# pytorch/ELF

Hardware: AMD Instinct MI355X
Metric: mcts_rollouts_per_sec (self-play, 19x19 Go, 8192 rollouts/move, bs 16) (higher is better)
Workload: dtype f32; 1 GPU; BASELINE configs[2]: MCTS self-play bs=16, 8192 rollouts/move, 20x256 fp16 net on PyTorch-ROCm, 2048 games/GPU in 1 group(s), window crosses a move boundary; games_per_gpu=2048, groups=1, board_size=19, mcts_threads=1, net_dtype=fp16, moves_in_window=2048, nodes_per_game=12288, node_bytes=6626, live_nodes=6241478, largest_tree=8184

## Files before the change

elf_amd/csrc/net_conv3x3.hip:

```cpp
#include <hip/hip_runtime.h>
#include <stdint.h>

#include "../../include/elf_amd.h"


namespace {

typedef _Float16 half8 __attribute__((ext_vector_type(8)));
typedef _Float16 half4 __attribute__((ext_vector_type(4)));
typedef float floatx16 __attribute__((ext_vector_type(16)));

constexpr int kTileM = 256;
constexpr int kTileN = 256;
constexpr int kThreads = 512;
constexpr int kOperandBytes = 256 * 128;
constexpr int kBufBytes = 2 * kOperandBytes;
constexpr int kLdsBytes = 2 * kBufBytes;

__device__ __attribute__((aligned(128))) unsigned char g_zero_line[128] = {0};

typedef const __attribute__((address_space(1))) void* gptr_t;
typedef __attribute__((address_space(3))) void* lptr_t;

__device__ __forceinline__ void stage16(const char* src, char* lds_base) {
  __builtin_amdgcn_global_load_lds((gptr_t)src, (lptr_t)lds_base, 16, 0, 0);
}

template <bool kHasRes>
__global__ __launch_bounds__(kThreads, 2) void k_conv3x3_f16(const char* __restrict__ x, const char* __restrict__ w,
                                                             const _Float16* __restrict__ bias, const _Float16* __restrict__ res,
                                                             _Float16* __restrict__ y, int M, int H, int W, int Cin, int K, int relu) {
  __shared__ __attribute__((aligned(128))) char lds[kLdsBytes];
  const int tid = threadIdx.x, lane = tid & 63, wv = tid >> 6;
  const int tile = blockIdx.x, kbase = blockIdx.y * kTileN;

  uint32_t xoff[4], woff[4], xmask[4];
  const unsigned char* zsrc = g_zero_line + (lane & 7) * 16;
#pragma unroll
  for (int i = 0; i < 4; ++i) {
    const int r = (i * 8 + wv) * 8 + (lane >> 3);
    const int chunk = (lane & 7) ^ ((r >> 1) & 7);
    const int p = tile * kTileM + r;
    uint32_t m = 0;
    if (p < M) {
      const int rem = p % (H * W), hh = rem / W, ww = rem - hh * W;
#pragma unroll
      for (int tap = 0; tap < 9; ++tap) {
        const int dy = tap / 3 - 1, dx = tap % 3 - 1;
        if ((unsigned)(hh + dy) < (unsigned)H && (unsigned)(ww + dx) < (unsigned)W) m |= 1u << tap;
      }
    }
    xmask[i] = m;
    xoff[i] = (uint32_t)p * (uint32_t)(Cin * 2) + chunk * 16;
    woff[i] = (uint32_t)(kbase + r) * (uint32_t)(9 * Cin * 2) + chunk * 16;
  }
  auto piece = [&](int j, int tap, int kc, int buf) {
    char* dst = lds + buf * kBufBytes + wv * 1024;
    if (j < 4) {
      const int dy = tap / 3 - 1, dx = tap - (tap / 3) * 3 - 1;
      const uint32_t d = (uint32_t)((dy * W + dx) * Cin * 2 + kc * 128);
      stage16(((xmask[j] >> tap) & 1) ? x + (uint32_t)(xoff[j] + d) : (const char*)zsrc, dst + j * 8192);
    } else {
      stage16(w + (uint32_t)(woff[j - 4] + (uint32_t)(tap * Cin * 2 + kc * 128)), dst + kOperandBytes + (j - 4) * 8192);
    }
  };

  const int wm = wv >> 2, wn = wv & 3;
  const int fr = lane & 31, fh = lane >> 5;
  const int sw = (fr >> 1) & 7;
  const int xrow = (wm * 128 + fr) * 128;
  const int wrow = kOperandBytes + (wn * 64 + fr) * 128;
  int cs[4];
#pragma unroll
  for (int kk = 0; kk < 4; ++kk) cs[kk] = (((kk >> 1) * 4 + fh * 2 + (kk & 1)) ^ sw) << 4;

  floatx16 acc[4][2];
#pragma unroll
  for (int mt = 0; mt < 4; ++mt)
#pragma unroll
    for (int nt = 0; nt < 2; ++nt)
#pragma unroll
      for (int e = 0; e < 16; ++e) acc[mt][nt][e] = 0.0f;

  const int kchunks = Cin >> 6, ktiles = 9 * kchunks;
#pragma unroll
  for (int j = 0; j < 8; ++j) piece(j, 0, 0, 0);
  int tap = 0, kc = 0;
  for (int t = 0; t < ktiles; ++t) {
    asm volatile("s_waitcnt vmcnt(0)" ::: "memory");
    __syncthreads();
    int ntap = tap, nkc = kc + 1;
    if (nkc == kchunks) { nkc = 0; ++ntap; }
    const bool more = t + 1 < ktiles;
    const int nbuf = (t + 1) & 1;
    tap = ntap; kc = nkc;
    const char* b = lds + (t & 1) * kBufBytes;
    half8 xf[2][4], wf[2][2];
#pragma unroll
    for (int nt = 0; nt < 2; ++nt) wf[0][nt] = *(const half8*)(b + wrow + nt * 4096 + cs[0]);
#pragma unroll
    for (int mt = 0; mt < 4; ++mt) xf[0][mt] = *(const half8*)(b + xrow + mt * 4096 + cs[0]);
#pragma unroll
    for (int kk = 0; kk < 4; ++kk) {
      const int cur = kk & 1, nxt = cur ^ 1;
      if (kk < 3) {
#pragma unroll
        for (int nt = 0; nt < 2; ++nt) wf[nxt][nt] = *(const half8*)(b + wrow + nt * 4096 + cs[kk + 1]);
#pragma unroll
        for (int mt = 0; mt < 4; ++mt) xf[nxt][mt] = *(const half8*)(b + xrow + mt * 4096 + cs[kk + 1]);
      }
      __builtin_amdgcn_sched_barrier(0);
#pragma unroll
      for (int mt = 0; mt < 2; ++mt)
#pragma unroll
        for (int nt = 0; nt < 2; ++nt)
          acc[mt][nt] = __builtin_amdgcn_mfma_f32_32x32x16_f16(wf[cur][nt], xf[cur][mt], acc[mt][nt], 0, 0, 0);
      __builtin_amdgcn_sched_barrier(0);
      if (more && kk < 2) { piece(4 * kk, ntap, nkc, nbuf); piece(4 * kk + 1, ntap, nkc, nbuf); }
      __builtin_amdgcn_sched_barrier(0);
#pragma unroll
      for (int mt = 2; mt < 4; ++mt)
#pragma unroll
        for (int nt = 0; nt < 2; ++nt)
          acc[mt][nt] = __builtin_amdgcn_mfma_f32_32x32x16_f16(wf[cur][nt], xf[cur][mt], acc[mt][nt], 0, 0, 0);
      __builtin_amdgcn_sched_barrier(0);
      if (more && kk < 2) { piece(4 * kk + 2, ntap, nkc, nbuf); piece(4 * kk + 3, ntap, nkc, nbuf); }
      __builtin_amdgcn_sched_barrier(0);
    }
  }

  __syncthreads();
#pragma unroll
  for (int mt = 0; mt < 4; ++mt)
#pragma unroll
    for (int nt = 0; nt < 2; ++nt) {
      const int pos = wm * 128 + mt * 32 + fr;
#pragma unroll
      for (int g = 0; g < 4; ++g) {
        const int ch = wn * 64 + nt * 32 + g * 8 + fh * 4;
        half4 hv;
#pragma unroll
        for (int e = 0; e < 4; ++e) hv[e] = (_Float16)acc[mt][nt][g * 4 + e];
        *(half4*)(lds + pos * 512 + (((ch >> 3) ^ (pos & 31)) << 4) + ((ch >> 2) & 1) * 8) = hv;
      }
    }
  const int q = tid & 31;
  const half8 bv = *(const half8*)(bias + kbase + q * 8);
  if constexpr (kHasRes) {
    half8 rv[16];
#pragma unroll
    for (int it = 0; it < 16; ++it) {
      const int p = tile * kTileM + it * 16 + (tid >> 5);
      rv[it] = *(const half8*)(res + (size_t)(p < M ? p : M - 1) * K + kbase + q * 8);
    }
    __syncthreads();
#pragma unroll
    for (int it = 0; it < 16; ++it) {
      const int pos = it * 16 + (tid >> 5);
      const int p = tile * kTileM + pos;
      const half8 cv = *(const half8*)(lds + pos * 512 + ((q ^ (pos & 31)) << 4));
      half8 ov;
#pragma unroll
      for (int e = 0; e < 8; ++e) {
        float v = (float)cv[e];
        v += (float)bv[e];
        v += (float)rv[it][e];
        if (relu) v = fmaxf(v, 0.0f);
        ov[e] = (_Float16)v;
      }
      if (p < M) *(half8*)(y + (size_t)p * K + kbase + q * 8) = ov;
    }
  } else {
    __syncthreads();
#pragma unroll 4
    for (int it = 0; it < 16; ++it) {
      const int pos = it * 16 + (tid >> 5);
      const int p = tile * kTileM + pos;
      if (p < M) {
        const half8 cv = *(const half8*)(lds + pos * 512 + ((q ^ (pos & 31)) << 4));
        half8 ov;
#pragma unroll
        for (int e = 0; e < 8; ++e) {
          float v = (float)cv[e];
          v += (float)bv[e];
          if (relu) v = fmaxf(v, 0.0f);
          ov[e] = (_Float16)v;
        }
        *(half8*)(y + (size_t)p * K + kbase + q * 8) = ov;
      }
    }
  }
}

}

extern "C" __attribute__((visibility("hidden"))) int elfnet_conv3x3_native_f16(const void* x, const void* w, const void* bias,
                                                                               const void* res, void* y, int64_t rows, int h, int wd,
                                                                               int c, int k, int relu, hipStream_t stream) {
  if ((c & 63) != 0 || (k & 255) != 0) return ELFGO_E_BADARG;
  const int64_t m = rows * h * wd;
  const dim3 grid((unsigned)((m + kTileM - 1) / kTileM), (unsigned)(k / kTileN));
  if (res)
    hipLaunchKernelGGL(k_conv3x3_f16<true>, grid, dim3(kThreads), 0, stream, (const char*)x, (const char*)w, (const _Float16*)bias,
                       (const _Float16*)res, (_Float16*)y, (int)m, h, wd, c, k, relu);
  else
    hipLaunchKernelGGL(k_conv3x3_f16<false>, grid, dim3(kThreads), 0, stream, (const char*)x, (const char*)w, (const _Float16*)bias,
                       (const _Float16*)nullptr, (_Float16*)y, (int)m, h, wd, c, k, relu);
  hipError_t e = hipGetLastError();
  return e == hipSuccess ? 0 : (int)e;
}
```

Measured before the change: 59540 rollouts/s.

## Restructure conv3x3 main loop into ping-pong staged pipeline with split wave groups

Rewrites the 3x3 conv GEMM main loop so that operand staging into LDS is split into half-tile pieces. The pieces are issued between two MFMA phases with partial vmcnt waits instead of a full drain each k-tile. The two wave halves are offset by one barrier, a ping-pong schedule in which one group computes while the other loads. MFMA sections run at raised priority, and the staging layout is remapped so each half of the tile arrives independently. This targets the load-wait stalls at every k-tile boundary, but the barrier and vmcnt logic is fragile and brings a risk of races or deadlock if the counts are wrong.

Result: faster. 61890 rollouts/s, median of 6 (+3.9%).

```diff
diff --git a/elf_amd/csrc/net_conv3x3.hip b/elf_amd/csrc/net_conv3x3.hip
--- a/elf_amd/csrc/net_conv3x3.hip
+++ b/elf_amd/csrc/net_conv3x3.hip
@@ -26,20 +26,33 @@
   __builtin_amdgcn_global_load_lds((gptr_t)src, (lptr_t)lds_base, 16, 0, 0);
 }
 
+template <int kN, bool kLgkm>
+__device__ __forceinline__ void wait_staged() {
+  if constexpr (kLgkm) asm volatile("s_waitcnt vmcnt(%0) lgkmcnt(0)" ::"n"(kN) : "memory");
+  else asm volatile("s_waitcnt vmcnt(%0)" ::"n"(kN) : "memory");
+}
+__device__ __forceinline__ void raw_barrier() {
+  __builtin_amdgcn_s_barrier();
+  asm volatile("" ::: "memory");
+  __builtin_amdgcn_sched_barrier(0);
+}
+template <int kV> struct Mode { static constexpr int v = kV; };
+
 template <bool kHasRes>
 __global__ __launch_bounds__(kThreads, 2) void k_conv3x3_f16(const char* __restrict__ x, const char* __restrict__ w,
                                                              const _Float16* __restrict__ bias, const _Float16* __restrict__ res,
                                                              _Float16* __restrict__ y, int M, int H, int W, int Cin, int K, int relu) {
   __shared__ __attribute__((aligned(128))) char lds[kLdsBytes];
-  const int tid = threadIdx.x, lane = tid & 63, wv = tid >> 6;
-  const int tile = blockIdx.x, kbase = blockIdx.y * kTileN;
+  const int tid = threadIdx.x, lane = tid & 63, wv = __builtin_amdgcn_readfirstlane(tid >> 6);
+  const int kbase = blockIdx.y * kTileN;
+  const int tile = blockIdx.x;
 
   uint32_t xoff[4], woff[4], xmask[4];
   const unsigned char* zsrc = g_zero_line + (lane & 7) * 16;
 #pragma unroll
-  for (int i = 0; i < 4; ++i) {
-    const int r = (i * 8 + wv) * 8 + (lane >> 3);
-    const int chunk = (lane & 7) ^ ((r >> 1) & 7);
+  for (int j = 0; j < 4; ++j) {
+    const int hf = j >> 1, i = j & 1;
+    const int r = i * 128 + hf * 64 + wv * 8 + (lane >> 3);
     const int p = tile * kTileM + r;
     uint32_t m = 0;
     if (p < M) {
@@ -50,19 +63,25 @@
         if ((unsigned)(hh + dy) < (unsigned)H && (unsigned)(ww + dx) < (unsigned)W) m |= 1u << tap;
       }
     }
-    xmask[i] = m;
-    xoff[i] = (uint32_t)p * (uint32_t)(Cin * 2) + chunk * 16;
-    woff[i] = (uint32_t)(kbase + r) * (uint32_t)(9 * Cin * 2) + chunk * 16;
+    xmask[j] = m;
+    xoff[j] = (uint32_t)p * (uint32_t)(Cin * 2) + (((lane & 7) ^ ((r >> 1) & 7)) << 4);
+    const int rw = (i * 2 + (wv >> 2)) * 64 + hf * 32 + (wv & 3) * 8 + (lane >> 3);
+    woff[j] = (uint32_t)(kbase + rw) * (uint32_t)(9 * Cin * 2) + (((lane & 7) ^ ((rw >> 1) & 7)) << 4);
   }
-  auto piece = [&](int j, int tap, int kc, int buf) {
-    char* dst = lds + buf * kBufBytes + wv * 1024;
-    if (j < 4) {
-      const int dy = tap / 3 - 1, dx = tap - (tap / 3) * 3 - 1;
-      const uint32_t d = (uint32_t)((dy * W + dx) * Cin * 2 + kc * 128);
-      stage16(((xmask[j] >> tap) & 1) ? x + (uint32_t)(xoff[j] + d) : (const char*)zsrc, dst + j * 8192);
-    } else {
-      stage16(w + (uint32_t)(woff[j - 4] + (uint32_t)(tap * Cin * 2 + kc * 128)), dst + kOperandBytes + (j - 4) * 8192);
-    }
+  auto stage_x = [&](int hf, int tap, int kc, int buf) {
+    const int dy = tap / 3 - 1, dx = tap - (tap / 3) * 3 - 1;
+    const uint32_t d = (uint32_t)((dy * W + dx) * Cin * 2 + kc * 128);
+#pragma unroll
+    for (int i = 0; i < 2; ++i)
+      stage16(((xmask[hf * 2 + i] >> tap) & 1) ? x + (uint32_t)(xoff[hf * 2 + i] + d) : (const char*)zsrc,
+              lds + buf * kBufBytes + (i * 128 + hf * 64 + wv * 8) * 128);
+  };
+  auto stage_w = [&](int hf, int tap, int kc, int buf) {
+    const uint32_t d = (uint32_t)(tap * Cin * 2 + kc * 128);
+#pragma unroll
+    for (int i = 0; i < 2; ++i)
+      stage16(w + (uint32_t)(woff[hf * 2 + i] + d),
+              lds + buf * kBufBytes + kOperandBytes + ((i * 2 + (wv >> 2)) * 64 + hf * 32 + (wv & 3) * 8) * 128);
   };
 
   const int wm = wv >> 2, wn = wv & 3;
@@ -73,6 +92,8 @@
   int cs[4];
 #pragma unroll
   for (int kk = 0; kk < 4; ++kk) cs[kk] = (((kk >> 1) * 4 + fh * 2 + (kk & 1)) ^ sw) << 4;
+  auto ldx = [&](const char* b, int mt, int kk) { return *(const half8*)(b + xrow + mt * 4096 + cs[kk]); };
+  auto ldw = [&](const char* b, int nt, int kk) { return *(const half8*)(b + wrow + nt * 4096 + cs[kk]); };
 
   floatx16 acc[4][2];
 #pragma unroll
@@ -83,51 +104,70 @@
       for (int e = 0; e < 16; ++e) acc[mt][nt][e] = 0.0f;
 
   const int kchunks = Cin >> 6, ktiles = 9 * kchunks;
-#pragma unroll
-  for (int j = 0; j < 8; ++j) piece(j, 0, 0, 0);
-  int tap = 0, kc = 0;
-  for (int t = 0; t < ktiles; ++t) {
-    asm volatile("s_waitcnt vmcnt(0)" ::: "memory");
-    __syncthreads();
-    int ntap = tap, nkc = kc + 1;
-    if (nkc == kchunks) { nkc = 0; ++ntap; }
-    const bool more = t + 1 < ktiles;
-    const int nbuf = (t + 1) & 1;
-    tap = ntap; kc = nkc;
-    const char* b = lds + (t & 1) * kBufBytes;
-    half8 xf[2][4], wf[2][2];
-#pragma unroll
-    for (int nt = 0; nt < 2; ++nt) wf[0][nt] = *(const half8*)(b + wrow + nt * 4096 + cs[0]);
-#pragma unroll
-    for (int mt = 0; mt < 4; ++mt) xf[0][mt] = *(const half8*)(b + xrow + mt * 4096 + cs[0]);
-#pragma unroll
-    for (int kk = 0; kk < 4; ++kk) {
-      const int cur = kk & 1, nxt = cur ^ 1;
-      if (kk < 3) {
-#pragma unroll
-        for (int nt = 0; nt < 2; ++nt) wf[nxt][nt] = *(const half8*)(b + wrow + nt * 4096 + cs[kk + 1]);
-#pragma unroll
-        for (int mt = 0; mt < 4; ++mt) xf[nxt][mt] = *(const half8*)(b + xrow + mt * 4096 + cs[kk + 1]);
-      }
-      __builtin_amdgcn_sched_barrier(0);
-#pragma unroll
-      for (int mt = 0; mt < 2; ++mt)
-#pragma unroll
-        for (int nt = 0; nt < 2; ++nt)
-          acc[mt][nt] = __builtin_amdgcn_mfma_f32_32x32x16_f16(wf[cur][nt], xf[cur][mt], acc[mt][nt], 0, 0, 0);
-      __builtin_amdgcn_sched_barrier(0);
-      if (more && kk < 2) { piece(4 * kk, ntap, nkc, nbuf); piece(4 * kk + 1, ntap, nkc, nbuf); }
-      __builtin_amdgcn_sched_barrier(0);
-#pragma unroll
-      for (int mt = 2; mt < 4; ++mt)
-#pragma unroll
-        for (int nt = 0; nt < 2; ++nt)
-          acc[mt][nt] = __builtin_amdgcn_mfma_f32_32x32x16_f16(wf[cur][nt], xf[cur][mt], acc[mt][nt], 0, 0, 0);
-      __builtin_amdgcn_sched_barrier(0);
-      if (more && kk < 2) { piece(4 * kk + 2, ntap, nkc, nbuf); piece(4 * kk + 3, ntap, nkc, nbuf); }
-      __builtin_amdgcn_sched_barrier(0);
-    }
+  half8 xf[2][4], wa[4], wb[4];
+  int tap1 = 0, kc1 = 1, tap2 = 0, kc2 = 2;
+  if (kchunks == 1) { tap1 = 1; kc1 = 0; tap2 = 2; kc2 = 0; }
+  else if (kchunks == 2) { tap2 = 1; kc2 = 0; }
+  stage_x(0, 0, 0, 0); stage_w(0, 0, 0, 0); stage_w(1, 0, 0, 0); stage_x(1, 0, 0, 0);
+  stage_x(0, tap1, kc1, 1); stage_w(0, tap1, kc1, 1); stage_w(1, tap1, kc1, 1);
+  wait_staged<8, false>();
+  raw_barrier();
+
+  auto ktile = [&](auto mode, int t) {
+    constexpr int kMode = decltype(mode)::v;
+    const int cur = t & 1, nxt = cur ^ 1;
+    const char* b = lds + cur * kBufBytes;
+#pragma unroll
+    for (int kk = 0; kk < 4; ++kk) {
+      wa[kk] = ldw(b, 0, kk);
+      xf[0][kk] = ldx(b, 0, kk);
+      xf[1][kk] = ldx(b, 1, kk);
+      wb[kk] = ldw(b, 1, kk);
+    }
+    if constexpr (kMode <= 1) stage_x(1, tap1, kc1, nxt);
+    wait_staged<kMode == 2 ? 0 : 8, true>();
+    raw_barrier();
+    __builtin_amdgcn_s_setprio(1);
+#pragma unroll
+    for (int kk = 0; kk < 4; ++kk) {
+      acc[0][0] = __builtin_amdgcn_mfma_f32_32x32x16_f16(wa[kk], xf[0][kk], acc[0][0], 0, 0, 0);
+      acc[1][0] = __builtin_amdgcn_mfma_f32_32x32x16_f16(wa[kk], xf[1][kk], acc[1][0], 0, 0, 0);
+      acc[0][1] = __builtin_amdgcn_mfma_f32_32x32x16_f16(wb[kk], xf[0][kk], acc[0][1], 0, 0, 0);
+      acc[1][1] = __builtin_amdgcn_mfma_f32_32x32x16_f16(wb[kk], xf[1][kk], acc[1][1], 0, 0, 0);
+    }
+    __builtin_amdgcn_s_setprio(0);
+    __builtin_amdgcn_sched_barrier(0);
+    raw_barrier();
+#pragma unroll
+    for (int kk = 0; kk < 4; ++kk) {
+      xf[0][kk] = ldx(b, 2, kk);
+      xf[1][kk] = ldx(b, 3, kk);
+    }
+    if constexpr (kMode == 0) { stage_x(0, tap2, kc2, cur); stage_w(0, tap2, kc2, cur); stage_w(1, tap2, kc2, cur); }
+    wait_staged<kMode == 0 ? 8 : kMode == 1 ? 2 : 0, true>();
+    raw_barrier();
+    __builtin_amdgcn_s_setprio(1);
+#pragma unroll
+    for (int kk = 0; kk < 4; ++kk) {
+      acc[2][0] = __builtin_amdgcn_mfma_f32_32x32x16_f16(wa[kk], xf[0][kk], acc[2][0], 0, 0, 0);
+      acc[3][0] = __builtin_amdgcn_mfma_f32_32x32x16_f16(wa[kk], xf[1][kk], acc[3][0], 0, 0, 0);
+      acc[2][1] = __builtin_amdgcn_mfma_f32_32x32x16_f16(wb[kk], xf[0][kk], acc[2][1], 0, 0, 0);
+      acc[3][1] = __builtin_amdgcn_mfma_f32_32x32x16_f16(wb[kk], xf[1][kk], acc[3][1], 0, 0, 0);
+    }
+    __builtin_amdgcn_s_setprio(0);
+    __builtin_amdgcn_sched_barrier(0);
+    raw_barrier();
+  };
+  const int late = __builtin_amdgcn_readfirstlane(tid >> 8);
+  if (late) raw_barrier();
+  for (int t = 0; t < ktiles - 2; ++t) {
+    ktile(Mode<0>{}, t);
+    tap1 = tap2; kc1 = kc2;
+    if (++kc2 == kchunks) { kc2 = 0; ++tap2; }
   }
+  ktile(Mode<1>{}, ktiles - 2);
+  ktile(Mode<2>{}, ktiles - 1);
+  if (!late) raw_barrier();
 
   __syncthreads();
 #pragma unroll
```
